# strukturag/libheif

Measured on NVIDIA H100. Metric: megapixels/sec HEIC-grid decode->RGB, higher is better.
Workload: dtype u8

## Files before the change

### libheif_b200/csrc/b200_hevc.h

```cpp
#pragma once
#include "b200_internal.h"
#include "b200_hevc_types.h"
#include "b200_hevc_syntax.h"
#include "b200_hevc_scaling.h"
#include <vector>

namespace b200 {

struct ParseLimits { uint64_t max_image_size_pixels = 0; };

struct PictureHeaders {
  PicDesc desc;
  syn::SeqParams sp;
  std::vector<SliceInfo> slices;
  std::vector<syn::Substream> subs;
  std::vector<uint8_t> rbsp;
  std::vector<uint16_t> ctu_slice;
  int colour_primaries = 2, transfer_characteristics = 2, matrix_coefficients = 2, full_range = 0;
  bool scaling_enabled = false;
  sl::Factors scaling;
};

struct ParsedPicture {
  PictureHeaders hdr;
// ... 15 lines not shown
  const int8_t* qp8; const uint8_t* edge8;
  const uint8_t* scaling;
  unsigned int* progress;
  const unsigned int* entropy_progress;
  int blocks_per_sm;
  unsigned int* ticket;
  unsigned int* error_flag;
  const uint2* row_list;
  int nrows;
  int wide_samples;
  int max_log2_ctb;
};
enum { MAX_CHUNKS = 16 };
struct EntropyPic { syn::SeqParams sp; syn::PicBuffers pb; uint32_t progress_base, sub_base; };
struct EntropyBatch {
  const EntropyPic* pics; int npics;
  const syn::Substream* subs;
  int nsubs;
  unsigned int* queue; unsigned int* qhead; unsigned int* qtail; unsigned int* deps;
  unsigned int* progress; unsigned int* sub_done; unsigned int* error_flag;
  int blocks_per_sm;
  int common;
};
int launch_entropy(const EntropyBatch& b, cudaStream_t s, int* resident_warps = nullptr);
int launch_entropy_gate(const EntropyBatch& b, int resident_warps, cudaStream_t s);
int launch_entropy_stats(const EntropyBatch& b, unsigned long long* out2, cudaStream_t s);
int launch_recon(const DeviceBatch& b, cudaStream_t s);
int launch_deblock(const DeviceBatch& b, const PicDesc* host_pics, cudaStream_t s);
int launch_sao(const DeviceBatch& b, const PicDesc* host_pics, cudaStream_t s, int* launches = nullptr);

}
```

### libheif_b200/csrc/b200_hevc_decode.cu

```cuda
#include "b200_hevc.h"
#include "b200_staging.h"
#include <chrono>
#include <functional>
#include <memory>
#include <mutex>
#include <string>
#include <unistd.h>

using namespace b200;

namespace {

double now_ms() { return std::chrono::duration<double, std::milli>(std::chrono::steady_clock::now().time_since_epoch()).count(); }

struct ScratchLayout {
  size_t n_rows = 0, n_subs = 0;
  static constexpr size_t error_flag = 1, progress = 2;
  size_t tickets() const { return progress + 3 * n_rows; }
  size_t sync_size() const { return tickets() + MAX_CHUNKS; }
  static constexpr size_t entropy_progress = 1;
  size_t sub_done() const { return entropy_progress + n_rows; }
  size_t esync_size() const { return sub_done() + n_subs; }
  static constexpr size_t qhead = 0, qtail = 1, queue = 2;
  size_t deps() const { return queue + n_subs; }
// ... 23 lines not shown
  bool device_front_end = false;
  size_t n_subs = 0;
  bool any_tiles = false;
  bool all_common = false;
  int bands = 0;
};

enum { OVERLAP_K0_BLOCKS_PER_SM = 3, OVERLAP_K1_BLOCKS_PER_SM = 2 };

struct LaunchPlan {
  int bands = 1, rows_per_band = 1;
  bool banded = false;
  bool overlap = false;
  bool tail = false;
  int k0_blocks_per_sm = 0, k1_blocks_per_sm = 0;
  bool common_k0 = false;
};

int sm_count() { int dev = 0, sms = 148; cudaGetDevice(&dev); cudaDeviceGetAttribute(&sms, cudaDevAttrMultiProcessorCount, dev); return sms; }

LaunchPlan plan_launches(const BatchShape& b, bool hook, const Overrides& env) {
  LaunchPlan p;
  const bool devfe = b.device_front_end;
  const bool one_wave = devfe && (env.overlap == Overrides::AUTO ? b.n_subs <= (size_t)sm_count() * 16
                                                                  : env.overlap == Overrides::ON);
  p.bands = b.bands;
  if (!p.bands) {
    p.bands = 1; p.rows_per_band = b.rows;
    if (b.rows >= 2 && (env.bands != Overrides::AUTO ? env.bands == Overrides::ON : hook && !one_wave)) {
      const int target = env.band_tiles > 0 ? env.band_tiles : (b.cols * b.rows + 1) / 2;
      int rpb = std::max(1, (target + b.cols / 2) / b.cols);
      if ((b.rows + rpb - 1) / rpb > MAX_CHUNKS) rpb = (b.rows + MAX_CHUNKS - 1) / MAX_CHUNKS;
      p.rows_per_band = rpb; p.bands = (b.rows + rpb - 1) / rpb;
    }
  }
  p.banded = p.bands > 1 && (hook || env.bands == Overrides::ON);
  p.overlap = !p.banded && one_wave;
  p.tail = devfe && env.overlap == Overrides::AUTO && env.tail && (!p.overlap || env.tail_force);
  if (p.tail) p.overlap = true;
  if (b.any_tiles) p.overlap = p.tail = false;
  if (p.overlap && !p.tail) { p.k0_blocks_per_sm = OVERLAP_K0_BLOCKS_PER_SM; p.k1_blocks_per_sm = OVERLAP_K1_BLOCKS_PER_SM; }
  p.common_k0 = b.all_common;
  return p;
}

}

// ... 706 lines not shown
```

### libheif_b200/csrc/b200_hevc_entropy.cu

```cuda
#include <cstdint>
#include <cstdlib>
namespace b200 { namespace syn {
__shared__ uint32_t s_kLps4[64];
__shared__ uint8_t s_kTransLps[64];
__shared__ uint8_t s_kNextState[256];
__shared__ unsigned long long s_kState[128];
__shared__ uint8_t s_kInitI[135];
__shared__ uint8_t s_kSigMap4[16];
__shared__ uint8_t s_kScanPos[3][16];
__shared__ uint8_t s_kScanInv[3][16];
__shared__ uint8_t s_kSbInv[4][3][64];
__shared__ uint8_t s_kSigCtx4[3][16];
__shared__ uint8_t s_kSigCtxN[3][4][16];
__shared__ uint8_t s_kChromaTab[4];
__shared__ uint8_t s_kScanX[4][3][64];
__shared__ uint8_t s_kScanY[4][3][64];
} }
#ifdef __CUDA_ARCH__
#define B200_T(name) s_##name
#endif
#include "b200_hevc.h"
static_assert(b200::syn::CTX_COUNT == 135, "s_kInitI above is sized for 135 context variables");

namespace b200 {
// ... 25 lines not shown
      if (e_ld_acquire(p) >= need) return;
      if ((++spins & 63u) != 0) continue;
      if (e_ld_acquire(error_flag)) return;
      if (spins > (1u << 23)) { atomicExch(error_flag, 3u); return; }
    }
  }
  __device__ void wait_row(int row, int need) { spin_until(progress + row, (unsigned)need, error_flag); }
  __device__ void publish_row(int row, int done) { e_st_release(progress + row, (unsigned)done); }
  __device__ void wait_substream(int idx) { spin_until(sub_done + idx, 1u, error_flag); }
  __device__ void finish_substream(int idx, int err) {
    e_st_release(sub_done + idx, 1u);
    if (err) atomicExch(error_flag, (unsigned)err);
  }
  __device__ void notify(int target) {
    if (target < 0) return;
    __threadfence();
    if (atomicSub(deps + target, 1u) == 1u) { const unsigned s = atomicAdd(qtail, 1u); e_st_release(queue + s, (unsigned)target + 1u); }
  }
};

#ifndef B200_ENTROPY_MIN_BLOCKS
#define B200_ENTROPY_MIN_BLOCKS 1
#endif
template <class Cfg>
__global__ void __launch_bounds__(EWARPS * 32, B200_ENTROPY_MIN_BLOCKS) hevc_entropy_kernel(const EntropyBatch b) {
  __shared__ __align__(8) syn::U2 s_ctx[EWARPS][syn::CTX_COUNT];
  __shared__ syn::DecoderT<Cfg> s_dec[EWARPS];
  for (int i = threadIdx.x; i < 64; i += blockDim.x) { syn::s_kLps4[i] = syn::d_kLps4[i]; syn::s_kTransLps[i] = syn::d_kTransLps[i]; }
  for (int i = threadIdx.x; i < syn::CTX_COUNT; i += blockDim.x) syn::s_kInitI[i] = syn::d_kInitI[i];
  for (int i = threadIdx.x; i < 256; i += blockDim.x) syn::s_kNextState[i] = syn::d_kNextState[i];
  for (int i = threadIdx.x; i < 128; i += blockDim.x) syn::s_kState[i] = syn::d_kState[i];
  for (int i = threadIdx.x; i < 16; i += blockDim.x) syn::s_kSigMap4[i] = syn::d_kSigMap4[i];
  for (int i = threadIdx.x; i < 48; i += blockDim.x) { (&syn::s_kScanPos[0][0])[i] = (&syn::d_kScanPos[0][0])[i]; (&syn::s_kScanInv[0][0])[i] = (&syn::d_kScanInv[0][0])[i]; (&syn::s_kSigCtx4[0][0])[i] = (&syn::d_kSigCtx4[0][0])[i]; }
  for (int i = threadIdx.x; i < 192; i += blockDim.x) (&syn::s_kSigCtxN[0][0][0])[i] = (&syn::d_kSigCtxN[0][0][0])[i];
  for (int i = threadIdx.x; i < 768; i += blockDim.x) (&syn::s_kSbInv[0][0][0])[i] = (&syn::d_kSbInv[0][0][0])[i];
  for (int i = threadIdx.x; i < 4; i += blockDim.x) syn::s_kChromaTab[i] = syn::d_kChromaTab[i];
  for (int i = threadIdx.x; i < 4 * 3 * 64; i += blockDim.x) { (&syn::s_kScanX[0][0][0])[i] = (&syn::d_kScanX[0][0][0])[i]; (&syn::s_kScanY[0][0][0])[i] = (&syn::d_kScanY[0][0][0])[i]; }
  __syncthreads();
  if ((threadIdx.x & 31) != 0) return;
  const int slot_w = threadIdx.x >> 5;
  const syn::CtxPtr ctx = (syn::CtxPtr)__cvta_generic_to_shared(s_ctx[slot_w]);
  for (;;) {
    const unsigned slot = atomicAdd(b.qhead, 1u);
    if (slot >= (unsigned)b.nsubs) break;
    unsigned item = e_ld_acquire(b.queue + slot);
    if (!item) {
      unsigned ns = 500, spins = 0;
      for (;;) {
        __nanosleep(ns); if (ns < 16000) ns <<= 1;
        if ((item = e_ld_acquire(b.queue + slot)) != 0u) break;
        if ((++spins & 31u) != 0) continue;
        if (e_ld_acquire(b.error_flag)) return;
        if (spins > (1u << 22)) { atomicExch(b.error_flag, 3u); return; }
      }
    }
    const syn::Substream& gs = b.subs[item - 1u];
    const EntropyPic& ep = b.pics[gs.pic];
    DevSync sync;
    sync.progress = b.progress + ep.progress_base; sync.sub_done = b.sub_done + ep.sub_base; sync.error_flag = b.error_flag;
    sync.queue = b.queue; sync.qtail = b.qtail; sync.deps = b.deps;
    sync.dense_tu = sync.dense_coef = sync.dense_tu_cap = sync.dense_coef_cap = 0; sync.end_bit_position = 0;
    syn::run_substream<Cfg>(s_dec[slot_w], ep.sp, ep.pb, b.subs + ep.sub_base, (int)(item - 1u - ep.sub_base), ctx, sync);
  }
}

__global__ void entropy_stats_kernel(const EntropyBatch b, unsigned long long* out2) {
  const int pi = blockIdx.y;
  const EntropyPic& ep = b.pics[pi];
  const int nctb = ep.sp.wctb * ep.sp.hctb;
  unsigned long long tus = 0, coefs = 0;
  for (int a = blockIdx.x * blockDim.x + threadIdx.x; a < nctb; a += gridDim.x * blockDim.x) {
    const CtuInfo ci = ep.pb.ctus[a];
    tus += ci.tu_count;
    for (unsigned k = 0; k < ci.tu_count; k++) { const TuCmd t = ep.pb.tus[ci.tu_start + k]; coefs += (t.w3 & 0x7ff) + ((t.w3 >> 11) & 0x3ff) + ((t.w3 >> 21) & 0x3ff); }
  }
  atomicAdd(out2, tus); atomicAdd(out2 + 1, coefs);
}

__global__ void entropy_gate_kernel(const unsigned* qhead, unsigned need, const unsigned* error_flag) {
  for (unsigned spins = 0; spins < 2000000u; spins++) {
    if (e_ld_acquire(qhead) >= need || e_ld_acquire(error_flag)) return;
    __nanosleep(1000);
  }
}

int launch_entropy_gate(const EntropyBatch& b, int resident_warps, cudaStream_t s) {
  if (b.nsubs <= 0 || resident_warps <= 0) return B200_OK;
  entropy_gate_kernel<<<1, 1, 0, s>>>(b.qhead, (unsigned)(resident_warps < b.nsubs ? resident_warps : b.nsubs), b.error_flag);
  cudaError_t e = cudaGetLastError();
  if (e != cudaSuccess) return set_error(B200_E_CUDA, "entropy gate launch: %s", cudaGetErrorString(e));
  return B200_OK;
}

int launch_entropy(const EntropyBatch& b, cudaStream_t s, int* resident_warps) {
  if (resident_warps) *resident_warps = 0;
  if (b.nsubs <= 0) return B200_OK;
  int dev = 0, sms = 148; cudaGetDevice(&dev); cudaDeviceGetAttribute(&sms, cudaDevAttrMultiProcessorCount, dev);
  auto kern = b.common ? hevc_entropy_kernel<syn::CfgCommon> : hevc_entropy_kernel<syn::CfgRuntime>;
  int occ = 1; cudaOccupancyMaxActiveBlocksPerMultiprocessor(&occ, kern, EWARPS * 32, 0);
  if (occ < 1) occ = 1;
  if (b.blocks_per_sm > 0 && b.blocks_per_sm < occ) occ = b.blocks_per_sm;
  const int want = (b.nsubs + EWARPS - 1) / EWARPS;
  const int grid = want < sms * occ ? want : sms * occ;
  if (resident_warps) *resident_warps = grid * EWARPS;
  kern<<<grid, EWARPS * 32, 0, s>>>(b);
  cudaError_t e = cudaGetLastError();
  if (e != cudaSuccess) return set_error(B200_E_CUDA, "entropy launch: %s", cudaGetErrorString(e));
  return B200_OK;
}

int launch_entropy_stats(const EntropyBatch& b, unsigned long long* out2, cudaStream_t s) {
  if (b.npics <= 0) return B200_OK;
  entropy_stats_kernel<<<dim3(8, b.npics), 128, 0, s>>>(b, out2);
  cudaError_t e = cudaGetLastError();
  if (e != cudaSuccess) return set_error(B200_E_CUDA, "entropy stats launch: %s", cudaGetErrorString(e));
  return B200_OK;
}

}
```

### libheif_b200/csrc/b200_hevc_syntax.h

```cpp
#pragma once
#include <cstdint>
#include <cstring>
#include "b200_hevc_types.h"

#if defined(__CUDA_ARCH__) && !defined(B200_SYNTAX_HOST_ONLY)
#define B200_SYN_DEVICE 1
#endif
#if defined(__CUDACC__) && !defined(B200_SYNTAX_HOST_ONLY)
#define B200_HDN __host__ __device__ __noinline__
#define B200_NOUNROLL _Pragma("unroll 1")
#define B200_HD __host__ __device__
#define B200_HDI __host__ __device__ __forceinline__
#define B200_TABLE(type, name, dims, ...) static const type h_##name dims = __VA_ARGS__; static __device__ const type d_##name dims = __VA_ARGS__;
#else
#define B200_HDN
#define B200_NOUNROLL
#define B200_HD
#define B200_HDI inline
#define B200_TABLE(type, name, dims, ...) static const type h_##name dims = __VA_ARGS__;
#endif
#if defined(B200_SYN_DEVICE) && !defined(B200_T)
#define B200_T(name) d_##name
#endif
#ifdef B200_SYN_DEVICE
// ... 215 lines not shown
  }
}

enum { SYN_OK = 0, SYN_E_BITSTREAM = 1, SYN_E_OVERFLOW = 2 };

struct SaoRaw { int8_t type[3], band[3], eo[3]; int8_t off[3][4]; };

struct CfgRuntime { enum : int { chroma = -1, bd = -1, log2_min_cb = -1, log2_min_tb = -1, log2_max_tb = -1, transform_skip = -1, cu_qp_delta = -1, sign_hiding = -1, sao_enabled = -1, wpp = -1, dense = -1, pcm = -1, tq_bypass = -1, tiles = -1 }; };
struct CfgCommon { enum : int { chroma = 1, bd = 8, log2_min_cb = 3, log2_min_tb = 2, log2_max_tb = 5, transform_skip = 0, cu_qp_delta = 1, sign_hiding = 1, sao_enabled = 1, wpp = 1, dense = 0, pcm = 0, tq_bypass = 0, tiles = 0 }; };
B200_HD inline bool matches_common(const SeqParams& q) {
  return q.chroma == 1 && q.bd == 8 && q.log2_min_cb == 3 && q.log2_min_tb == 2 && q.log2_max_tb == 5 && !q.transform_skip && q.cu_qp_delta == 1 && q.sign_hiding == 1 &&
         q.sao_enabled == 1 && q.wpp == 1 && q.dense == 0 && !q.pcm && !q.tq_bypass && !q.tiles;
}
#define B200_SPC(f) ((int)Cfg::f >= 0 ? (int)Cfg::f : (int)sp->f)
#define B200_SPR(f) ((int)Cfg::f >= 0 ? (int)Cfg::f : (int)sp.f)

template <class Cfg>
struct DecoderT {
  const SeqParams* sp; PicBuffers pb; const Substream* ss;
  Cabac cabac; CabacStream stream; CtxPtr ctx;
  int is_dqp_coded, dqp_val, qpy_prev_qg, last_cu_qpy, first_qg, cur_qpy, err;
  int cu_bypass;
  uint32_t tu_n, coef_n, tu_cap, coef_cap;
  int cur_ctb_x, cur_ctb_y;
  int ctb_x0, ctb_y0, left_ok, up_ok;
  int left_lf, up_lf;
  struct Cu { int x0, y0, log2cb, nxn, lmode[4], cmode; int cmodes[4]; };

  B200_HD inline bool avail(int x, int y) const { return x >= ctb_x0 ? (y >= ctb_y0 ? true : up_ok != 0) : left_ok != 0; }
  B200_HD inline int ld_cell(const uint8_t* p, int y) const { return y >= ctb_y0 ? (int)*p : (int)B200_LD_SHARED(p); }

  B200_HDN int dbin(int ci) { return cabac.bin(ctx_at(ctx, ci), stream); }
  B200_HDN int dbypass() { return cabac.bypass(stream); }
  B200_HDN unsigned dbits(int k) { return cabac.bypass_bits(k, stream); }

  B200_HDN void parse_sao(int rx, int ry, CtuInfo& ci) {
    const int addr = ry * sp->wctb + rx;
    B200_NOUNROLL for (int c = 0; c < 3; c++) { ci.sao[c].type = 0; ci.sao[c].band_or_class = 0; B200_NOUNROLL for (int k = 0; k < 4; k++) ci.sao[c].offset[k] = 0; }
    if (!ss->sao_luma && !ss->sao_chroma) return;
    int ml = 0, mu = 0;
    if (left_ok) ml = dbin(CTX_SAO_MERGE);
    if (up_ok && !ml) mu = dbin(CTX_SAO_MERGE);
    if (ml || mu) {
      const unsigned long long* o = reinterpret_cast<const unsigned long long*>(pb.ctus[ml ? addr - 1 : addr - sp->wctb].sao);
      unsigned long long* dsto = reinterpret_cast<unsigned long long*>(ci.sao);
      B200_NOUNROLL for (int c = 0; c < 3; c++) dsto[c] = B200_LD_SHARED(o + c);
// ... 13 lines not shown
        B200_NOUNROLL for (int i = 0; i < 4; i++) ci.sao[c].offset[i] = (int8_t)clip3(-128, 127, av[i] * (1 << sc));
      } else {
        if (c < 2) ci.sao[c].band_or_class = (uint8_t)dbits(2); else ci.sao[2].band_or_class = ci.sao[1].band_or_class;
        ci.sao[c].offset[0] = (int8_t)clip3(-128, 127, av[0] << sc); ci.sao[c].offset[1] = (int8_t)clip3(-128, 127, av[1] << sc);
        ci.sao[c].offset[2] = (int8_t)clip3(-128, 127, -(av[2] << sc)); ci.sao[c].offset[3] = (int8_t)clip3(-128, 127, -(av[3] << sc));
      }
    }
  }

  B200_HDN void derive_qpy(int xcb, int ycb) {
    const int mask = (1 << sp->qg_log2) - 1, xqg = xcb & ~mask, yqg = ycb & ~mask, cm = ~((1 << sp->log2ctb) - 1);
    int qa = qpy_prev_qg, qb = qpy_prev_qg;
    if (avail(xqg - 1, yqg) && ((xqg - 1) & cm) == (xqg & cm)) qa = pb.qp8[(yqg >> 3) * sp->w8 + ((xqg - 1) >> 3)];
    if (avail(xqg, yqg - 1) && ((yqg - 1) & cm) == (yqg & cm)) qb = pb.qp8[((yqg - 1) >> 3) * sp->w8 + (xqg >> 3)];
    const int pred = (qa + qb + 1) >> 1, qbd = 6 * (B200_SPC(bd) - 8);
    cur_qpy = ((pred + dqp_val + 52 + 2 * qbd) % (52 + qbd)) - qbd;
  }

  B200_HDN int residual(int log2n, int c, int mode, int& tskip) {
    const int n = 1 << log2n;
    Cabac cb_ = cabac; const CtxPtr cx = ctx;
    const int bypass_cu = B200_SPC(tq_bypass) && cu_bypass;
    const int sign_hiding = B200_SPC(sign_hiding) && !bypass_cu;
    CoefEntry* const coef_out = pb.coefs; uint32_t cn = coef_n; const uint32_t ccap = coef_cap;
    tskip = 0;
    if (B200_SPC(transform_skip) && log2n == 2 && !bypass_cu) tskip = cb_.bin(ctx_at(cx, CTX_TSKIP + (c ? 1 : 0)), stream);
    const int cmax = (log2n << 1) - 1;
    int off, shift;
    if (c == 0) { off = 3 * (log2n - 2) + ((log2n - 1) >> 2); shift = (log2n + 1) >> 2; } else { off = 15; shift = log2n - 2; }
    int lx = 0, ly = 0;
    B200_NOUNROLL for (int xy = 0; xy < 2; xy++) {
      const CtxPtr lc = ctx_at(cx, (xy ? CTX_LAST_Y : CTX_LAST_X) + off);
      int l = 0;
      CtxPtr a_cur = lc; U2 e_cur = ctx_ld(a_cur);
      B200_NOUNROLL while (l < cmax) {
        const CtxPtr a_next = ctx_at(lc, (l + 1) >> shift);
        U2 e_next = ctx_ld(a_next), ne;
        const int b = cb_.bin_e(e_cur, a_cur, stream, ne);
        if (!b) break;
        if (a_next == a_cur) e_next = ne;
        a_cur = a_next; e_cur = e_next; l++;
      }
      if (xy) ly = l; else lx = l;
    }
    B200_NOUNROLL for (int xy = 0; xy < 2; xy++) {
      int l = xy ? ly : lx;
      if (l > 3) { const int nb = (l >> 1) - 1; l = (1 << nb) * (2 + (l & 1)) + (int)cb_.bypass_bits(nb, stream); }
      if (xy) ly = l; else lx = l;
    }
    int scan = 0;
    if (log2n == 2 || (log2n == 3 && (c == 0 || B200_SPC(chroma) == 3))) { if (mode >= 6 && mode <= 14) scan = 2; else if (mode >= 22 && mode <= 30) scan = 1; }
    if (scan == 2) { const int t = lx; lx = ly; ly = t; }
    if (lx >= n || ly >= n) { err = SYN_E_BITSTREAM; cabac = cb_; return 0; }
    const int l2sb = log2n - 2;
    const uint8_t *sbx = B200_T(kScanX)[l2sb][scan], *sby = B200_T(kScanY)[l2sb][scan], *spos = B200_T(kScanPos)[scan];
    const int last_sb = B200_T(kSbInv)[l2sb][scan][((ly >> 2) << 3) + (lx >> 2)];
    const int last_pos = B200_T(kScanInv)[scan][((ly & 3) << 2) + (lx & 3)];
    uint64_t csbf = 0;
    int carry = 1, count = 0; bool first_done = false;
    const int nsbw = 1 << l2sb;
    const int dc_ctx = CTX_SIG + (c ? 27 : 0);
    const int sig_base = log2n == 2 ? dc_ctx : (c == 0 ? CTX_SIG + (log2n == 3 ? (scan == 0 ? 9 : 15) : 21) : CTX_SIG + 27 + (log2n == 3 ? 9 : 12));
    B200_NOUNROLL for (int i = last_sb; i >= 0; i--) {
      const int xs = sbx[i], ys = sby[i];
      const int right = (xs + 1 < nsbw) ? (int)((csbf >> (ys * 8 + xs + 1)) & 1) : 0;
      const int below = (ys + 1 < nsbw) ? (int)((csbf >> ((ys + 1) * 8 + xs)) & 1) : 0;
      int infer_dc = 0;
      if (i < last_sb && i > 0) { if (!cb_.bin(ctx_at(cx, CTX_CSBF + ((right | below) ? 1 : 0) + (c ? 2 : 0)), stream)) continue; infer_dc = 1; }
      csbf |= 1ull << (ys * 8 + xs);
      const TabPtr tab = log2n == 2 ? B200_TADDR(kSigCtx4) + 16 * scan : B200_TADDR(kSigCtxN) + (64 * scan + 16 * (right | (below << 1)));
      const CtxPtr cbase = ctx_at(cx, sig_base + ((c == 0 && log2n > 2 && (xs | ys)) ? 3 : 0));
      unsigned sig = 0;
      int k = 15;
      if (i == last_sb) { sig = 1u; k = last_pos - 1; }
      if (k >= 0) {
        const CtxPtr a0 = i == 0 ? ctx_at(cx, dc_ctx) : ctx_at(cbase, (int)tab_ld8(tab, 0));
        CtxPtr a_cur = k > 0 ? ctx_at(cbase, (int)tab_ld8(tab, k)) : a0;
        U2 e_cur = ctx_ld(a_cur);
        B200_NOUNROLL for (; k > 0; k--) {
          const CtxPtr a_next = k > 1 ? ctx_at(cbase, (int)tab_ld8(tab, k - 1)) : a0;
          U2 e_next = ctx_ld(a_next), ne;
          sig = (sig << 1) | (unsigned)cb_.bin_e(e_cur, a_cur, stream, ne);
          if (a_next == a_cur) e_next = ne;
          a_cur = a_next; e_cur = e_next;
        }
        if (infer_dc && !sig) sig = 1u;
        else { U2 ne; sig = (sig << 1) | (unsigned)cb_.bin_e(e_cur, a_cur, stream, ne); }
      }
      if (!sig) continue;
      unsigned g1 = 0;
      int g1ctx = 1, g2 = 0;
      int ctx_set = (i == 0 || c > 0) ? 0 : 2;
      if (first_done && carry == 0) ctx_set++;
      first_done = true;
      const int last_sig = hi_bit(sig), first_sig = lo_bit(sig);
      { unsigned m = sig; const CtxPtr gbase = ctx_at(cx, CTX_GT1 + ctx_set * 4 + (c ? 16 : 0));
        B200_NOUNROLL for (int ng1 = 0; m && ng1 < 8; ng1++) {
          const int kk = hi_bit(m); m ^= 1u << kk;
          if (cb_.bin(ctx_at(gbase, imin(3, g1ctx)), stream)) { g1 |= 1u << kk; g1ctx = 0; } else if (g1ctx > 0) g1ctx++;
        } }
      carry = g1ctx;
      const int last_g1 = g1 ? hi_bit(g1) : -1;
      const bool hidden = sign_hiding && (last_sig - first_sig > 3);
      if (last_g1 >= 0) g2 = cb_.bin(ctx_at(cx, CTX_GT2 + ctx_set + (c ? 4 : 0)), stream);
      const int nsign = pop_count(sig) - (hidden ? 1 : 0);
      const unsigned signs = cb_.bypass_bits(nsign, stream);
      int nsig = 0, sum = 0, rice = 0, sidx = nsign;
      B200_NOUNROLL for (unsigned m = sig; m; nsig++) {
        const int kk = hi_bit(m); m ^= 1u << kk;
        const int base = 1 + (int)((g1 >> kk) & 1) + (kk == last_g1 ? g2 : 0);
        int a = base;
        if (base == ((nsig < 8) ? ((kk == last_g1) ? 3 : 2) : 1)) {
          int pre = 0; B200_NOUNROLL while (pre < 32 && cb_.bypass(stream)) pre++;
          if (pre > 20) { err = SYN_E_BITSTREAM; cabac = cb_; coef_n = cn; return count; }
          const int rem = (pre <= 3 ? (pre << rice) : (((1 << (pre - 3)) + 3 - 1) << rice)) + (int)cb_.bypass_bits(pre <= 3 ? rice : pre - 3 + rice, stream);
          a = base + rem;
          if (a > 3 * (1 << rice)) rice = imin(rice + 1, 4);
        }
        int neg = 0;
        if (!hidden || kk != first_sig) { sidx--; neg = (int)((signs >> sidx) & 1); }
        int v = neg ? -a : a;
        if (hidden) { sum += a; if (kk == first_sig && (sum & 1)) v = -v; }
        if (cn >= ccap) { err = SYN_E_OVERFLOW; cabac = cb_; coef_n = cn; return count; }
        const int p = spos[kk];
        CoefEntry e; e.pos = (uint16_t)((((ys << 2) + (p >> 2)) << log2n) + (xs << 2) + (p & 3)); e.level = (int16_t)clip3(-32768, 32767, v);
        coef_out[cn++] = e; count++;
      }
    }
    cabac = cb_; coef_n = cn;
    return count;
  }

  B200_HDN void mark_tu(int x0, int y0, int log2n) {
    const SliceInfo& sl = pb.slices[ss->slice_idx];
    const int n8 = log2n > 3 ? 1 << (log2n - 3) : 1, bx = x0 >> 3, by = y0 >> 3;
    uint8_t left = 0, top = 0;
    if (!sl.deblocking_disabled) {
      if ((x0 & 7) == 0 && x0 > 0 && (x0 > ctb_x0 || left_lf)) left = 1;
      if ((y0 & 7) == 0 && y0 > 0 && (y0 > ctb_y0 || up_lf)) top = 2;
    }
    uint8_t* e = pb.edge8 + by * sp->w8 + bx;
    if (left) B200_NOUNROLL for (int y = 0; y < n8; y++) e[y * sp->w8] |= left;
    if (top) B200_NOUNROLL for (int x = 0; x < n8; x++) e[x] |= top;
  }

  B200_HDI void transform_unit(const Cu& cu, int x0, int y0, int log2n, int blk, int cbf_l, int cbf_cb, int cbf_cr, int pcb, int pcr) {
    const int cbf_c = B200_SPC(chroma) ? (log2n > 2 ? (cbf_cb | cbf_cr) : (pcb | pcr)) : 0;
    if ((cbf_l || cbf_c) && B200_SPC(cu_qp_delta) && !is_dqp_coded) {
      int v = 0;
      B200_NOUNROLL while (v < 5 && dbin(CTX_QP_DELTA + (v ? 1 : 0))) v++;
      if (v == 5) { int k = 0; B200_NOUNROLL while (k < 16 && dbypass()) { v += 1 << k; k++; } v += (int)dbits(k); }
      if (v && dbypass()) v = -v;
      { const int half = 3 * (B200_SPC(bd) - 8); if (v < -(26 + half) || v > 25 + half) { err = SYN_E_BITSTREAM; return; } }
      is_dqp_coded = 1; dqp_val = v;
      derive_qpy(cu.x0, cu.y0);
    }
    const int pu = cu.nxn ? ((y0 >= cu.y0 + (1 << (cu.log2cb - 1))) ? 2 : 0) + ((x0 >= cu.x0 + (1 << (cu.log2cb - 1))) ? 1 : 0) : 0;
    const int lmode = cu.lmode[pu];
    const uint32_t coef0 = coef_n;
    int ts_l = 0, ts_cb = 0, ts_cr = 0, nl = 0, ncb = 0, ncr = 0;
    int chroma_here = 0, ccb = 0, ccr = 0;
    if (B200_SPC(chroma)) {
      if (log2n > 2) { chroma_here = 1; ccb = cbf_cb; ccr = cbf_cr; }
      else if (blk == 3) { chroma_here = 1; ccb = pcb; ccr = pcr; }
    }
    B200_NOUNROLL for (int c = 0; c < 3; c++) {
      const int coded = c == 0 ? cbf_l : (c == 1 ? ccb : ccr);
      if (!coded) continue;
      int ts = 0;
      const int cnt = residual(c == 0 ? log2n : (log2n > 2 ? log2n - 1 : 2), c, c == 0 ? lmode : cu.cmode, ts);
      if (c == 0) { nl = cnt; ts_l = ts; } else if (c == 1) { ncb = cnt; ts_cb = ts; } else { ncr = cnt; ts_cr = ts; }
    }
    mark_tu(x0, y0, log2n);
    if (tu_n >= tu_cap) { err = SYN_E_OVERFLOW; return; }
    TuCmd t;
    t.w0 = (uint32_t)(x0 >> 2) | ((uint32_t)(y0 >> 2) << 12) | ((uint32_t)(log2n - 2) << 24) | ((uint32_t)cbf_l << 26) | ((uint32_t)ccb << 27) |
           ((uint32_t)ccr << 28) | ((uint32_t)chroma_here << 29) | ((uint32_t)ts_l << 30) | ((uint32_t)ts_cb << 31);
    t.w1 = (uint32_t)lmode | ((uint32_t)cu.cmode << 6) | ((uint32_t)(cur_qpy + 64) << 12) | ((uint32_t)ts_cr << 20) | ((B200_SPC(tq_bypass) && cu_bypass) ? 1u << 22 : 0u);
    t.w2 = coef0;
    t.w3 = (uint32_t)nl | ((uint32_t)ncb << 11) | ((uint32_t)ncr << 21);
    pb.tus[tu_n++] = t;
  }

  B200_HD static inline int zx(unsigned i) { i &= 0x55u; i = (i | (i >> 1)) & 0x33u; i = (i | (i >> 2)) & 0x0fu; return (int)i; }
  B200_HD static inline int node_depth(unsigned i, int levels) { const int up = i ? lo_bit(i) >> 1 : levels; return levels - imin(up, levels); }

  B200_HDI void transform_tree(const Cu& cu, int max_depth) {
    const int levels = cu.log2cb - 2, total = 1 << (2 * levels);
    unsigned cbm = 0, crm = 0;
    B200_NOUNROLL for (int j = 0; j < total && !err;) {
      int depth = node_depth((unsigned)j, levels);
      B200_NOUNROLL for (;;) {
        const int log2n = cu.log2cb - depth;
        const int x0 = cu.x0 + (zx((unsigned)j) << 2), y0 = cu.y0 + (zx((unsigned)j >> 1) << 2);
        const int blk = depth ? (j >> (2 * (levels - depth))) & 3 : 0;
        const int pcb = depth ? (int)((cbm >> (depth - 1)) & 1) : 0, pcr = depth ? (int)((crm >> (depth - 1)) & 1) : 0;
        int split;
        if (log2n <= B200_SPC(log2_max_tb) && log2n > B200_SPC(log2_min_tb) && depth < max_depth && !(cu.nxn && depth == 0)) split = dbin(CTX_SPLIT_TR + 5 - log2n);
        else split = (log2n > B200_SPC(log2_max_tb) || (cu.nxn && depth == 0)) ? 1 : 0;
        if (split && log2n <= 2) { err = SYN_E_BITSTREAM; break; }
        int cb = 0, cr = 0;
        if (B200_SPC(chroma)) {
          if (log2n > 2) {
// ... 189 lines not shown
    if (B200_SPC(pcm) && !cu.nxn && log2cb >= sp->log2_min_pcm && log2cb <= sp->log2_max_pcm && cabac.terminate(stream)) { pcm_unit(x0, y0, log2cb, depth); return; }
    const int np = cu.nxn ? 4 : 1, pbs = cu.nxn ? n / 2 : n;
    int prev[4], mi[4] = {0, 0, 0, 0}, rem[4] = {0, 0, 0, 0};
    B200_NOUNROLL for (int i = 0; i < np; i++) prev[i] = dbin(CTX_PREV_INTRA);
    B200_NOUNROLL for (int i = 0; i < np; i++) { if (prev[i]) { mi[i] = dbypass(); if (mi[i]) mi[i] += dbypass(); } else rem[i] = (int)dbits(5); }
    B200_NOUNROLL for (int i = 0; i < np; i++) {
      const int px = x0 + (i & 1) * pbs, py = y0 + (i >> 1) * pbs;
      const int m = luma_mode(px, py, prev[i], mi[i], rem[i]);
      cu.lmode[i] = m;
      B200_NOUNROLL for (int yy = 0; yy < pbs; yy += 4) B200_NOUNROLL for (int xx = 0; xx < pbs; xx += 4) pb.ipm4[((py + yy) >> 2) * sp->w4 + ((px + xx) >> 2)] = (uint8_t)m;
    }
    if (B200_SPC(chroma) >= 2) chroma_modes_x(cu, np);
    else if (B200_SPC(chroma)) {
      int v = 4; if (dbin(CTX_CHROMA_PRED)) v = (int)dbits(2);
      if (v == 4) cu.cmode = cu.lmode[0]; else { cu.cmode = B200_T(kChromaTab)[v]; if (cu.cmode == cu.lmode[0]) cu.cmode = 34; }
    }
    B200_NOUNROLL for (int yy = 0; yy < n; yy += 8) B200_NOUNROLL for (int xx = 0; xx < n; xx += 8) pb.cd8[((y0 + yy) >> 3) * sp->w8 + ((x0 + xx) >> 3)] = (uint8_t)depth;
    if (!B200_SPC(cu_qp_delta)) cur_qpy = ss->slice_qp; else derive_qpy(x0, y0);
    if (B200_SPC(chroma) >= 2) transform_tree_x(cu, sp->max_th_depth_intra + cu.nxn); else transform_tree(cu, sp->max_th_depth_intra + cu.nxn);
    B200_NOUNROLL for (int yy = 0; yy < n; yy += 8) B200_NOUNROLL for (int xx = 0; xx < n; xx += 8) pb.qp8[((y0 + yy) >> 3) * sp->w8 + ((x0 + xx) >> 3)] = (int8_t)cur_qpy;
    last_cu_qpy = cur_qpy;
  }

  B200_HDI void coding_quadtree(int xc, int yc) {
    const int log2min = B200_SPC(log2_min_cb), levels = sp->log2ctb - log2min, total = 1 << (2 * levels);
    B200_NOUNROLL for (int i = 0; i < total && !err;) {
      int depth = node_depth((unsigned)i, levels);
      B200_NOUNROLL for (;;) {
        const int log2cb = sp->log2ctb - depth, n = 1 << log2cb;
        const int x0 = xc + (zx((unsigned)i) << log2min), y0 = yc + (zx((unsigned)i >> 1) << log2min);
        if (x0 >= sp->W || y0 >= sp->H) { i += 1 << (2 * (levels - depth)); break; }
        int split;
        if (x0 + n <= sp->W && y0 + n <= sp->H && log2cb > log2min) {
          int inc = 0;
          if (avail(x0 - 1, y0) && (int)pb.cd8[(y0 >> 3) * sp->w8 + ((x0 - 1) >> 3)] > depth) inc++;
          if (avail(x0, y0 - 1) && ld_cell(pb.cd8 + ((y0 - 1) >> 3) * sp->w8 + (x0 >> 3), y0 - 1) > depth) inc++;
          split = dbin(CTX_SPLIT_CU + inc);
        } else split = log2cb > log2min;
        if (B200_SPC(cu_qp_delta) && log2cb >= sp->qg_log2) {
          is_dqp_coded = 0; dqp_val = 0;
          if (!split || log2cb == sp->qg_log2) { if (first_qg) { qpy_prev_qg = ss->slice_qp; first_qg = 0; } else qpy_prev_qg = last_cu_qpy; }
        }
        if (split) { depth++; continue; }
        coding_unit(x0, y0, log2cb, depth);
        i += 1 << (2 * (levels - depth));
        break;
      }
    }
  }

  B200_HDN void decode_ctb(int addr) {
    const int rx = addr % sp->wctb, ry = addr / sp->wctb;
    cur_ctb_x = rx; cur_ctb_y = ry;
    ctb_x0 = rx << sp->log2ctb; ctb_y0 = ry << sp->log2ctb;
    left_ok = rx > 0 && pb.ctu_slice[addr - 1] == (uint16_t)ss->slice_idx;
    up_ok = ry > 0 && pb.ctu_slice[addr - sp->wctb] == (uint16_t)ss->slice_idx;
    {
      const SliceInfo& cs = pb.slices[ss->slice_idx];
      left_lf = left_ok; up_lf = up_ok;
      if (rx > 0 && !left_ok) { const SliceInfo& o = pb.slices[pb.ctu_slice[addr - 1]]; left_lf = (o.slice_id == cs.slice_id || cs.lf_across_slices) && (o.tile_id == cs.tile_id || cs.lf_across_tiles); }
      if (ry > 0 && !up_ok) { const SliceInfo& o = pb.slices[pb.ctu_slice[addr - sp->wctb]]; up_lf = (o.slice_id == cs.slice_id || cs.lf_across_slices) && (o.tile_id == cs.tile_id || cs.lf_across_tiles); } }
    CtuInfo& ci = pb.ctus[addr];
    ci.slice_idx = (uint16_t)ss->slice_idx;
    if (!B200_SPC(dense)) { tu_n = (uint32_t)addr * (uint32_t)sp->tu_slots; tu_cap = tu_n + (uint32_t)sp->tu_slots; coef_n = (uint32_t)addr * (uint32_t)sp->coef_slots; coef_cap = coef_n + (uint32_t)sp->coef_slots; }
    const uint32_t t0 = tu_n;
    if (B200_SPC(sao_enabled)) parse_sao(rx, ry, ci);
    else for (int c = 0; c < 3; c++) { ci.sao[c].type = 0; ci.sao[c].band_or_class = 0; B200_NOUNROLL for (int k = 0; k < 4; k++) ci.sao[c].offset[k] = 0; }
    { const int b0x = rx << (sp->log2ctb - 3), b0y = ry << (sp->log2ctb - 3), nb = 1 << (sp->log2ctb - 3);
      B200_NOUNROLL for (int y = 0; y < nb && b0y + y < sp->h8; y++) B200_NOUNROLL for (int x = 0; x < nb && b0x + x < sp->w8; x++) pb.edge8[(b0y + y) * sp->w8 + b0x + x] = 0; }
    coding_quadtree(rx << sp->log2ctb, ry << sp->log2ctb);
    ci.tu_start = t0; ci.tu_count = (uint16_t)(tu_n - t0);
  }
};

typedef DecoderT<CfgRuntime> Decoder;

template <class Cfg, class Sync>
B200_HD int run_substream(DecoderT<Cfg>& d, const SeqParams& sp, const PicBuffers& pb, const Substream* all, int index, CtxPtr ctx, Sync& sync) {
  const Substream& ss = all[index];
  d.sp = &sp; d.pb = pb; d.ss = &ss; d.ctx = ctx; d.err = SYN_OK;
  d.is_dqp_coded = 0; d.dqp_val = 0; d.qpy_prev_qg = ss.slice_qp; d.last_cu_qpy = ss.slice_qp; d.first_qg = 1; d.cur_qpy = ss.slice_qp; d.cu_bypass = 0;
  d.tu_n = 0; d.coef_n = 0; d.tu_cap = 0; d.coef_cap = 0;
  if (B200_SPR(dense)) {
    d.tu_n = sync.dense_tu; d.coef_n = sync.dense_coef; d.tu_cap = sync.dense_tu_cap; d.coef_cap = sync.dense_coef_cap;
  }
  const int rx0 = (int)(ss.ctb_begin % (uint32_t)sp.wctb), ry0 = (int)(ss.ctb_begin / (uint32_t)sp.wctb);
  if (ss.prev >= 0) {
    sync.wait_substream(ss.prev);
    const uint8_t* st = pb.end_state + (size_t)ss.prev * CTX_STRIDE;
    B200_NOUNROLL for (int i = 0; i < CTX_COUNT; i++) ctx_st(ctx_at(ctx, i), tab_ld64(B200_TADDR(kState), (int)B200_LD_SHARED(st + i) & 127));
    d.last_cu_qpy = (int)(int8_t)B200_LD_SHARED(st + CTX_COUNT); d.first_qg = 0;
  }
  if (ss.init_contexts) init_contexts(ctx, ss.slice_qp);
  if (B200_SPR(wpp) && rx0 == 0 && (!ss.init_contexts || ss.prev >= 0) && ss.ctb_begin != ss.slice_addr_rs) {
    const int xn = 1 << sp.log2ctb, yn = (ry0 - 1) << sp.log2ctb;
    bool tr = ry0 > 0 && xn < sp.W && pb.ctu_slice[(ry0 - 1) * sp.wctb + 1] == (uint16_t)ss.slice_idx;
    (void)yn;
    if (tr) { sync.wait_row(ry0 - 1, 2); const uint8_t* st = pb.wpp_ctx + (size_t)(ry0 - 1) * CTX_STRIDE; B200_NOUNROLL for (int i = 0; i < CTX_COUNT; i++) ctx_st(ctx_at(ctx, i), tab_ld64(B200_TADDR(kState), (int)B200_LD_SHARED(st + i) & 127)); }
    else if (ss.prev < 0) init_contexts(ctx, ss.slice_qp);
    d.first_qg = 1;
  }
  d.stream.d = pb.rbsp; d.stream.size = pb.rbsp_size;
  d.cabac.start(d.stream, ss.byte_begin);
  const bool tiles = B200_SPR(tiles) != 0;
  int rx = rx0, ry = ry0;
  const uint32_t nctb = ss.ctb_end - ss.ctb_begin;
  B200_NOUNROLL for (uint32_t k = 0; k < nctb; k++, rx++) {
    if (rx == (int)ss.tile_x1) { rx = (int)ss.tile_x0; ry++; }
    const uint32_t a = (uint32_t)ry * (uint32_t)sp.wctb + (uint32_t)rx;
    if (ry > 0 && !tiles) sync.wait_row(ry - 1, rx + 1);
    if (B200_SPR(wpp) && rx == 0 && a != ss.ctb_begin) {
      d.first_qg = 1;
    }
    if (!B200_SPR(wpp) && rx == 0 && a != ss.ctb_begin) {  }
    d.decode_ctb((int)a);
    if (d.err) break;
    if (B200_SPR(wpp) && rx == 1) { uint8_t* st = pb.wpp_ctx + (size_t)ry * CTX_STRIDE; B200_NOUNROLL for (int i = 0; i < CTX_COUNT; i++) st[i] = (uint8_t)(ctx_ld(ctx_at(ctx, i)).y >> 24); }
    const int end = d.cabac.terminate(d.stream);
    const bool last = k + 1 == nctb;
    if (end != ((last && ss.last_of_segment) ? 1 : 0)) { d.err = SYN_E_BITSTREAM; break; }
    if (last && !ss.last_of_segment) { if (!d.cabac.terminate(d.stream)) { d.err = SYN_E_BITSTREAM; break; } }
    if (!tiles) sync.publish_row(ry, rx + 1);
    if (B200_SPR(wpp) && rx == 1) sync.notify(ss.wake_ctb2);
    if (d.cabac.pos > pb.rbsp_size + 64u) { d.err = SYN_E_BITSTREAM; break; }
  }
  { uint8_t* st = pb.end_state + (size_t)index * CTX_STRIDE; B200_NOUNROLL for (int i = 0; i < CTX_COUNT; i++) st[i] = (uint8_t)(ctx_ld(ctx_at(ctx, i)).y >> 24); st[CTX_COUNT] = (uint8_t)(int8_t)d.last_cu_qpy; }
  if (B200_SPR(dense)) { sync.dense_tu = d.tu_n; sync.dense_coef = d.coef_n; }
  sync.end_bit_position = d.cabac.bit_position();
  sync.finish_substream(index, d.err);
  if (!d.err) sync.notify(ss.wake_end);
  return d.err;
}

}
}
```

Measured before the change: 3691.

## Cut entropy kernel register pressure and raise occupancy for common config

The entropy kernel's register footprint is reduced in several ways. Per-warp sync state moves to shared memory, and live locals in residual coding are dropped: the coefficient counter is derived from indices, scan tables go through tab pointers, and quadtree levels are recomputed. TU fields are packed directly into the command word, and the loop re-reads state from the decoder object. The common-config kernel gets a min-blocks launch bound of 5, and the overlap one-wave threshold now uses the actual occupancy-derived warps per SM instead of a fixed 16. Forcing more blocks can cause spills, and the altered one-wave test can flip between overlap and banded launch plans.

```diff
diff --git a/libheif_b200/csrc/b200_hevc.h b/libheif_b200/csrc/b200_hevc.h
--- a/libheif_b200/csrc/b200_hevc.h
+++ b/libheif_b200/csrc/b200_hevc.h
@@ -61,6 +61,7 @@
   int blocks_per_sm;
   int common;
 };
+int entropy_warps_per_sm(bool common);
 int launch_entropy(const EntropyBatch& b, cudaStream_t s, int* resident_warps = nullptr);
 int launch_entropy_gate(const EntropyBatch& b, int resident_warps, cudaStream_t s);
 int launch_entropy_stats(const EntropyBatch& b, unsigned long long* out2, cudaStream_t s);
diff --git a/libheif_b200/csrc/b200_hevc_decode.cu b/libheif_b200/csrc/b200_hevc_decode.cu
--- a/libheif_b200/csrc/b200_hevc_decode.cu
+++ b/libheif_b200/csrc/b200_hevc_decode.cu
@@ -69,7 +69,7 @@
 LaunchPlan plan_launches(const BatchShape& b, bool hook, const Overrides& env) {
   LaunchPlan p;
   const bool devfe = b.device_front_end;
-  const bool one_wave = devfe && (env.overlap == Overrides::AUTO ? b.n_subs <= (size_t)sm_count() * 16
+  const bool one_wave = devfe && (env.overlap == Overrides::AUTO ? b.n_subs <= (size_t)sm_count() * entropy_warps_per_sm(b.all_common)
                                                                   : env.overlap == Overrides::ON);
   p.bands = b.bands;
   if (!p.bands) {
diff --git a/libheif_b200/csrc/b200_hevc_entropy.cu b/libheif_b200/csrc/b200_hevc_entropy.cu
--- a/libheif_b200/csrc/b200_hevc_entropy.cu
+++ b/libheif_b200/csrc/b200_hevc_entropy.cu
@@ -71,10 +71,16 @@
 #ifndef B200_ENTROPY_MIN_BLOCKS
 #define B200_ENTROPY_MIN_BLOCKS 1
 #endif
+#ifndef B200_ENTROPY_MAX_BLOCKS_PER_SM
+#define B200_ENTROPY_MAX_BLOCKS_PER_SM 0
+#endif
+template <class Cfg> constexpr int entropy_min_blocks() { return B200_ENTROPY_MIN_BLOCKS; }
+template <> constexpr int entropy_min_blocks<syn::CfgCommon>() { return B200_ENTROPY_MIN_BLOCKS > 5 ? B200_ENTROPY_MIN_BLOCKS : 5; }
 template <class Cfg>
-__global__ void __launch_bounds__(EWARPS * 32, B200_ENTROPY_MIN_BLOCKS) hevc_entropy_kernel(const EntropyBatch b) {
+__global__ void __launch_bounds__(EWARPS * 32, entropy_min_blocks<Cfg>()) hevc_entropy_kernel(const EntropyBatch b) {
   __shared__ __align__(8) syn::U2 s_ctx[EWARPS][syn::CTX_COUNT];
   __shared__ syn::DecoderT<Cfg> s_dec[EWARPS];
+  __shared__ DevSync s_sync[EWARPS];
   for (int i = threadIdx.x; i < 64; i += blockDim.x) { syn::s_kLps4[i] = syn::d_kLps4[i]; syn::s_kTransLps[i] = syn::d_kTransLps[i]; }
   for (int i = threadIdx.x; i < syn::CTX_COUNT; i += blockDim.x) syn::s_kInitI[i] = syn::d_kInitI[i];
   for (int i = threadIdx.x; i < 256; i += blockDim.x) syn::s_kNextState[i] = syn::d_kNextState[i];
@@ -105,7 +111,7 @@
     }
     const syn::Substream& gs = b.subs[item - 1u];
     const EntropyPic& ep = b.pics[gs.pic];
-    DevSync sync;
+    DevSync& sync = s_sync[slot_w];
     sync.progress = b.progress + ep.progress_base; sync.sub_done = b.sub_done + ep.sub_base; sync.error_flag = b.error_flag;
     sync.queue = b.queue; sync.qtail = b.qtail; sync.deps = b.deps;
     sync.dense_tu = sync.dense_coef = sync.dense_tu_cap = sync.dense_coef_cap = 0; sync.end_bit_position = 0;
@@ -141,13 +147,22 @@
   return B200_OK;
 }
 
+static int entropy_blocks_per_sm(bool common) {
+  auto kern = common ? hevc_entropy_kernel<syn::CfgCommon> : hevc_entropy_kernel<syn::CfgRuntime>;
+  int occ = 1; cudaOccupancyMaxActiveBlocksPerMultiprocessor(&occ, kern, EWARPS * 32, 0);
+  if (occ < 1) occ = 1;
+  if (B200_ENTROPY_MAX_BLOCKS_PER_SM > 0 && occ > B200_ENTROPY_MAX_BLOCKS_PER_SM) occ = B200_ENTROPY_MAX_BLOCKS_PER_SM;
+  return occ;
+}
+
+int entropy_warps_per_sm(bool common) { return entropy_blocks_per_sm(common) * EWARPS; }
+
 int launch_entropy(const EntropyBatch& b, cudaStream_t s, int* resident_warps) {
   if (resident_warps) *resident_warps = 0;
   if (b.nsubs <= 0) return B200_OK;
   int dev = 0, sms = 148; cudaGetDevice(&dev); cudaDeviceGetAttribute(&sms, cudaDevAttrMultiProcessorCount, dev);
   auto kern = b.common ? hevc_entropy_kernel<syn::CfgCommon> : hevc_entropy_kernel<syn::CfgRuntime>;
-  int occ = 1; cudaOccupancyMaxActiveBlocksPerMultiprocessor(&occ, kern, EWARPS * 32, 0);
-  if (occ < 1) occ = 1;
+  int occ = entropy_blocks_per_sm(b.common != 0);
   if (b.blocks_per_sm > 0 && b.blocks_per_sm < occ) occ = b.blocks_per_sm;
   const int want = (b.nsubs + EWARPS - 1) / EWARPS;
   const int grid = want < sms * occ ? want : sms * occ;
diff --git a/libheif_b200/csrc/b200_hevc_syntax.h b/libheif_b200/csrc/b200_hevc_syntax.h
--- a/libheif_b200/csrc/b200_hevc_syntax.h
+++ b/libheif_b200/csrc/b200_hevc_syntax.h
@@ -261,6 +261,7 @@
   int is_dqp_coded, dqp_val, qpy_prev_qg, last_cu_qpy, first_qg, cur_qpy, err;
   int cu_bypass;
   uint32_t tu_n, coef_n, tu_cap, coef_cap;
+  uint32_t ctb_tu0;
   int cur_ctb_x, cur_ctb_y;
   int ctb_x0, ctb_y0, left_ok, up_ok;
   int left_lf, up_lf;
@@ -320,7 +321,7 @@
     Cabac cb_ = cabac; const CtxPtr cx = ctx;
     const int bypass_cu = B200_SPC(tq_bypass) && cu_bypass;
     const int sign_hiding = B200_SPC(sign_hiding) && !bypass_cu;
-    CoefEntry* const coef_out = pb.coefs; uint32_t cn = coef_n; const uint32_t ccap = coef_cap;
+    uint32_t cn = coef_n;
     tskip = 0;
     if (B200_SPC(transform_skip) && log2n == 2 && !bypass_cu) tskip = cb_.bin(ctx_at(cx, CTX_TSKIP + (c ? 1 : 0)), stream);
     const int cmax = (log2n << 1) - 1;
@@ -351,28 +352,27 @@
     if (scan == 2) { const int t = lx; lx = ly; ly = t; }
     if (lx >= n || ly >= n) { err = SYN_E_BITSTREAM; cabac = cb_; return 0; }
     const int l2sb = log2n - 2;
-    const uint8_t *sbx = B200_T(kScanX)[l2sb][scan], *sby = B200_T(kScanY)[l2sb][scan], *spos = B200_T(kScanPos)[scan];
+    const TabPtr sbx = B200_TADDR(kScanX) + 64 * (3 * l2sb + scan), sby = B200_TADDR(kScanY) + 64 * (3 * l2sb + scan), spos = B200_TADDR(kScanPos) + 16 * scan;
     const int last_sb = B200_T(kSbInv)[l2sb][scan][((ly >> 2) << 3) + (lx >> 2)];
     const int last_pos = B200_T(kScanInv)[scan][((ly & 3) << 2) + (lx & 3)];
     uint64_t csbf = 0;
-    int carry = 1, count = 0; bool first_done = false;
-    const int nsbw = 1 << l2sb;
-    const int dc_ctx = CTX_SIG + (c ? 27 : 0);
-    const int sig_base = log2n == 2 ? dc_ctx : (c == 0 ? CTX_SIG + (log2n == 3 ? (scan == 0 ? 9 : 15) : 21) : CTX_SIG + 27 + (log2n == 3 ? 9 : 12));
+    int carry = 1;
+    const int sig_base = log2n == 2 ? CTX_SIG + (c ? 27 : 0) : (c == 0 ? CTX_SIG + (log2n == 3 ? (scan == 0 ? 9 : 15) : 21) : CTX_SIG + 27 + (log2n == 3 ? 9 : 12));
     B200_NOUNROLL for (int i = last_sb; i >= 0; i--) {
-      const int xs = sbx[i], ys = sby[i];
-      const int right = (xs + 1 < nsbw) ? (int)((csbf >> (ys * 8 + xs + 1)) & 1) : 0;
-      const int below = (ys + 1 < nsbw) ? (int)((csbf >> ((ys + 1) * 8 + xs)) & 1) : 0;
+      const int xs = (int)tab_ld8(sbx, i), ys = (int)tab_ld8(sby, i);
+      const int right = ((xs + 1) >> l2sb) == 0 ? (int)((csbf >> (ys * 8 + xs + 1)) & 1) : 0;
+      const int below = ((ys + 1) >> l2sb) == 0 ? (int)((csbf >> ((ys + 1) * 8 + xs)) & 1) : 0;
+      const bool is_last = csbf == 0;
       int infer_dc = 0;
-      if (i < last_sb && i > 0) { if (!cb_.bin(ctx_at(cx, CTX_CSBF + ((right | below) ? 1 : 0) + (c ? 2 : 0)), stream)) continue; infer_dc = 1; }
+      if (!is_last && i > 0) { if (!cb_.bin(ctx_at(cx, CTX_CSBF + ((right | below) ? 1 : 0) + (c ? 2 : 0)), stream)) continue; infer_dc = 1; }
       csbf |= 1ull << (ys * 8 + xs);
       const TabPtr tab = log2n == 2 ? B200_TADDR(kSigCtx4) + 16 * scan : B200_TADDR(kSigCtxN) + (64 * scan + 16 * (right | (below << 1)));
       const CtxPtr cbase = ctx_at(cx, sig_base + ((c == 0 && log2n > 2 && (xs | ys)) ? 3 : 0));
       unsigned sig = 0;
       int k = 15;
-      if (i == last_sb) { sig = 1u; k = last_pos - 1; }
+      if (is_last) { sig = 1u; k = last_pos - 1; }
       if (k >= 0) {
-        const CtxPtr a0 = i == 0 ? ctx_at(cx, dc_ctx) : ctx_at(cbase, (int)tab_ld8(tab, 0));
+        const CtxPtr a0 = i == 0 ? ctx_at(cx, CTX_SIG + (c ? 27 : 0)) : ctx_at(cbase, (int)tab_ld8(tab, 0));
         CtxPtr a_cur = k > 0 ? ctx_at(cbase, (int)tab_ld8(tab, k)) : a0;
         U2 e_cur = ctx_ld(a_cur);
         B200_NOUNROLL for (; k > 0; k--) {
@@ -389,8 +389,7 @@
       unsigned g1 = 0;
       int g1ctx = 1, g2 = 0;
       int ctx_set = (i == 0 || c > 0) ? 0 : 2;
-      if (first_done && carry == 0) ctx_set++;
-      first_done = true;
+      if (carry == 0) ctx_set++;
       const int last_sig = hi_bit(sig), first_sig = lo_bit(sig);
       { unsigned m = sig; const CtxPtr gbase = ctx_at(cx, CTX_GT1 + ctx_set * 4 + (c ? 16 : 0));
         B200_NOUNROLL for (int ng1 = 0; m && ng1 < 8; ng1++) {
@@ -410,7 +409,7 @@
         int a = base;
         if (base == ((nsig < 8) ? ((kk == last_g1) ? 3 : 2) : 1)) {
           int pre = 0; B200_NOUNROLL while (pre < 32 && cb_.bypass(stream)) pre++;
-          if (pre > 20) { err = SYN_E_BITSTREAM; cabac = cb_; coef_n = cn; return count; }
+          if (pre > 20) { err = SYN_E_BITSTREAM; cabac = cb_; const int count = (int)(cn - coef_n); coef_n = cn; return count; }
           const int rem = (pre <= 3 ? (pre << rice) : (((1 << (pre - 3)) + 3 - 1) << rice)) + (int)cb_.bypass_bits(pre <= 3 ? rice : pre - 3 + rice, stream);
           a = base + rem;
           if (a > 3 * (1 << rice)) rice = imin(rice + 1, 4);
@@ -419,13 +418,15 @@
         if (!hidden || kk != first_sig) { sidx--; neg = (int)((signs >> sidx) & 1); }
         int v = neg ? -a : a;
         if (hidden) { sum += a; if (kk == first_sig && (sum & 1)) v = -v; }
-        if (cn >= ccap) { err = SYN_E_OVERFLOW; cabac = cb_; coef_n = cn; return count; }
-        const int p = spos[kk];
+        if (cn >= coef_cap) { err = SYN_E_OVERFLOW; cabac = cb_; const int count = (int)(cn - coef_n); coef_n = cn; return count; }
+        const int p = (int)tab_ld8(spos, kk);
         CoefEntry e; e.pos = (uint16_t)((((ys << 2) + (p >> 2)) << log2n) + (xs << 2) + (p & 3)); e.level = (int16_t)clip3(-32768, 32767, v);
-        coef_out[cn++] = e; count++;
-      }
-    }
-    cabac = cb_; coef_n = cn;
+        pb.coefs[cn++] = e;
+      }
+    }
+    cabac = cb_;
+    const int count = (int)(cn - coef_n);
+    coef_n = cn;
     return count;
   }
 
@@ -456,27 +457,28 @@
     const int pu = cu.nxn ? ((y0 >= cu.y0 + (1 << (cu.log2cb - 1))) ? 2 : 0) + ((x0 >= cu.x0 + (1 << (cu.log2cb - 1))) ? 1 : 0) : 0;
     const int lmode = cu.lmode[pu];
     const uint32_t coef0 = coef_n;
-    int ts_l = 0, ts_cb = 0, ts_cr = 0, nl = 0, ncb = 0, ncr = 0;
     int chroma_here = 0, ccb = 0, ccr = 0;
     if (B200_SPC(chroma)) {
       if (log2n > 2) { chroma_here = 1; ccb = cbf_cb; ccr = cbf_cr; }
       else if (blk == 3) { chroma_here = 1; ccb = pcb; ccr = pcr; }
     }
-    B200_NOUNROLL for (int c = 0; c < 3; c++) {
-      const int coded = c == 0 ? cbf_l : (c == 1 ? ccb : ccr);
-      if (!coded) continue;
-      int ts = 0;
-      const int cnt = residual(c == 0 ? log2n : (log2n > 2 ? log2n - 1 : 2), c, c == 0 ? lmode : cu.cmode, ts);
-      if (c == 0) { nl = cnt; ts_l = ts; } else if (c == 1) { ncb = cnt; ts_cb = ts; } else { ncr = cnt; ts_cr = ts; }
-    }
-    mark_tu(x0, y0, log2n);
-    if (tu_n >= tu_cap) { err = SYN_E_OVERFLOW; return; }
     TuCmd t;
     t.w0 = (uint32_t)(x0 >> 2) | ((uint32_t)(y0 >> 2) << 12) | ((uint32_t)(log2n - 2) << 24) | ((uint32_t)cbf_l << 26) | ((uint32_t)ccb << 27) |
-           ((uint32_t)ccr << 28) | ((uint32_t)chroma_here << 29) | ((uint32_t)ts_l << 30) | ((uint32_t)ts_cb << 31);
-    t.w1 = (uint32_t)lmode | ((uint32_t)cu.cmode << 6) | ((uint32_t)(cur_qpy + 64) << 12) | ((uint32_t)ts_cr << 20) | ((B200_SPC(tq_bypass) && cu_bypass) ? 1u << 22 : 0u);
+           ((uint32_t)ccr << 28) | ((uint32_t)chroma_here << 29);
+    t.w1 = (uint32_t)lmode | ((uint32_t)cu.cmode << 6) | ((B200_SPC(tq_bypass) && cu_bypass) ? 1u << 22 : 0u);
     t.w2 = coef0;
-    t.w3 = (uint32_t)nl | ((uint32_t)ncb << 11) | ((uint32_t)ncr << 21);
+    t.w3 = 0;
+    B200_NOUNROLL for (int c = 0; c < 3; c++) {
+      if (!((t.w0 >> (26 + c)) & 1u)) continue;
+      const int l2 = (int)((t.w0 >> 24) & 3u) + 2;
+      int ts = 0;
+      const int cnt = residual(c == 0 ? l2 : (l2 > 2 ? l2 - 1 : 2), c, (int)((t.w1 >> (c == 0 ? 0 : 6)) & 63u), ts);
+      t.w3 |= (uint32_t)cnt << (c == 0 ? 0 : (c == 1 ? 11 : 21));
+      if (c == 0) t.w0 |= (uint32_t)ts << 30; else if (c == 1) t.w0 |= (uint32_t)ts << 31; else t.w1 |= (uint32_t)ts << 20;
+    }
+    mark_tu((int)(t.w0 & 0xfffu) << 2, (int)((t.w0 >> 12) & 0xfffu) << 2, (int)((t.w0 >> 24) & 3u) + 2);
+    if (tu_n >= tu_cap) { err = SYN_E_OVERFLOW; return; }
+    t.w1 |= (uint32_t)(cur_qpy + 64) << 12;
     pb.tus[tu_n++] = t;
   }
 
@@ -712,14 +714,15 @@
     last_cu_qpy = cur_qpy;
   }
 
-  B200_HDI void coding_quadtree(int xc, int yc) {
-    const int log2min = B200_SPC(log2_min_cb), levels = sp->log2ctb - log2min, total = 1 << (2 * levels);
-    B200_NOUNROLL for (int i = 0; i < total && !err;) {
-      int depth = node_depth((unsigned)i, levels);
+  B200_HD inline int cq_levels() const { return sp->log2ctb - B200_SPC(log2_min_cb); }
+  B200_HDI void coding_quadtree() {
+    const int log2min = B200_SPC(log2_min_cb);
+    B200_NOUNROLL for (int i = 0; i < (1 << (2 * cq_levels())) && !err;) {
+      int depth = node_depth((unsigned)i, cq_levels());
       B200_NOUNROLL for (;;) {
         const int log2cb = sp->log2ctb - depth, n = 1 << log2cb;
-        const int x0 = xc + (zx((unsigned)i) << log2min), y0 = yc + (zx((unsigned)i >> 1) << log2min);
-        if (x0 >= sp->W || y0 >= sp->H) { i += 1 << (2 * (levels - depth)); break; }
+        const int x0 = ctb_x0 + (zx((unsigned)i) << log2min), y0 = ctb_y0 + (zx((unsigned)i >> 1) << log2min);
+        if (x0 >= sp->W || y0 >= sp->H) { i += 1 << (2 * (cq_levels() - depth)); break; }
         int split;
         if (x0 + n <= sp->W && y0 + n <= sp->H && log2cb > log2min) {
           int inc = 0;
@@ -733,7 +736,7 @@
         }
         if (split) { depth++; continue; }
         coding_unit(x0, y0, log2cb, depth);
-        i += 1 << (2 * (levels - depth));
+        i += 1 << (2 * (cq_levels() - depth));
         break;
       }
     }
@@ -753,13 +756,14 @@
     CtuInfo& ci = pb.ctus[addr];
     ci.slice_idx = (uint16_t)ss->slice_idx;
     if (!B200_SPC(dense)) { tu_n = (uint32_t)addr * (uint32_t)sp->tu_slots; tu_cap = tu_n + (uint32_t)sp->tu_slots; coef_n = (uint32_t)addr * (uint32_t)sp->coef_slots; coef_cap = coef_n + (uint32_t)sp->coef_slots; }
-    const uint32_t t0 = tu_n;
+    ctb_tu0 = tu_n;
     if (B200_SPC(sao_enabled)) parse_sao(rx, ry, ci);
     else for (int c = 0; c < 3; c++) { ci.sao[c].type = 0; ci.sao[c].band_or_class = 0; B200_NOUNROLL for (int k = 0; k < 4; k++) ci.sao[c].offset[k] = 0; }
     { const int b0x = rx << (sp->log2ctb - 3), b0y = ry << (sp->log2ctb - 3), nb = 1 << (sp->log2ctb - 3);
       B200_NOUNROLL for (int y = 0; y < nb && b0y + y < sp->h8; y++) B200_NOUNROLL for (int x = 0; x < nb && b0x + x < sp->w8; x++) pb.edge8[(b0y + y) * sp->w8 + b0x + x] = 0; }
-    coding_quadtree(rx << sp->log2ctb, ry << sp->log2ctb);
-    ci.tu_start = t0; ci.tu_count = (uint16_t)(tu_n - t0);
+    coding_quadtree();
+    CtuInfo& ce = pb.ctus[cur_ctb_y * sp->wctb + cur_ctb_x];
+    ce.tu_start = ctb_tu0; ce.tu_count = (uint16_t)(tu_n - ctb_tu0);
   }
 };
 
@@ -794,31 +798,30 @@
   d.cabac.start(d.stream, ss.byte_begin);
   const bool tiles = B200_SPR(tiles) != 0;
   int rx = rx0, ry = ry0;
-  const uint32_t nctb = ss.ctb_end - ss.ctb_begin;
-  B200_NOUNROLL for (uint32_t k = 0; k < nctb; k++, rx++) {
-    if (rx == (int)ss.tile_x1) { rx = (int)ss.tile_x0; ry++; }
-    const uint32_t a = (uint32_t)ry * (uint32_t)sp.wctb + (uint32_t)rx;
+  B200_NOUNROLL for (uint32_t left = ss.ctb_end - ss.ctb_begin; left > 0; left--, rx++) {
+    if (rx == (int)d.ss->tile_x1) { rx = (int)d.ss->tile_x0; ry++; }
+    const uint32_t a = (uint32_t)ry * (uint32_t)d.sp->wctb + (uint32_t)rx;
     if (ry > 0 && !tiles) sync.wait_row(ry - 1, rx + 1);
-    if (B200_SPR(wpp) && rx == 0 && a != ss.ctb_begin) {
+    if (B200_SPR(wpp) && rx == 0 && a != d.ss->ctb_begin) {
       d.first_qg = 1;
     }
-    if (!B200_SPR(wpp) && rx == 0 && a != ss.ctb_begin) {  }
     d.decode_ctb((int)a);
     if (d.err) break;
-    if (B200_SPR(wpp) && rx == 1) { uint8_t* st = pb.wpp_ctx + (size_t)ry * CTX_STRIDE; B200_NOUNROLL for (int i = 0; i < CTX_COUNT; i++) st[i] = (uint8_t)(ctx_ld(ctx_at(ctx, i)).y >> 24); }
+    rx = d.cur_ctb_x; ry = d.cur_ctb_y;
+    if (B200_SPR(wpp) && rx == 1) { uint8_t* st = d.pb.wpp_ctx + (size_t)ry * CTX_STRIDE; B200_NOUNROLL for (int i = 0; i < CTX_COUNT; i++) st[i] = (uint8_t)(ctx_ld(ctx_at(d.ctx, i)).y >> 24); }
     const int end = d.cabac.terminate(d.stream);
-    const bool last = k + 1 == nctb;
-    if (end != ((last && ss.last_of_segment) ? 1 : 0)) { d.err = SYN_E_BITSTREAM; break; }
-    if (last && !ss.last_of_segment) { if (!d.cabac.terminate(d.stream)) { d.err = SYN_E_BITSTREAM; break; } }
+    const bool last = left == 1;
+    if (end != ((last && d.ss->last_of_segment) ? 1 : 0)) { d.err = SYN_E_BITSTREAM; break; }
+    if (last && !d.ss->last_of_segment) { if (!d.cabac.terminate(d.stream)) { d.err = SYN_E_BITSTREAM; break; } }
     if (!tiles) sync.publish_row(ry, rx + 1);
-    if (B200_SPR(wpp) && rx == 1) sync.notify(ss.wake_ctb2);
-    if (d.cabac.pos > pb.rbsp_size + 64u) { d.err = SYN_E_BITSTREAM; break; }
-  }
-  { uint8_t* st = pb.end_state + (size_t)index * CTX_STRIDE; B200_NOUNROLL for (int i = 0; i < CTX_COUNT; i++) st[i] = (uint8_t)(ctx_ld(ctx_at(ctx, i)).y >> 24); st[CTX_COUNT] = (uint8_t)(int8_t)d.last_cu_qpy; }
+    if (B200_SPR(wpp) && rx == 1) sync.notify(d.ss->wake_ctb2);
+    if (d.cabac.pos > d.pb.rbsp_size + 64u) { d.err = SYN_E_BITSTREAM; break; }
+  }
+  { uint8_t* st = d.pb.end_state + (size_t)index * CTX_STRIDE; B200_NOUNROLL for (int i = 0; i < CTX_COUNT; i++) st[i] = (uint8_t)(ctx_ld(ctx_at(d.ctx, i)).y >> 24); st[CTX_COUNT] = (uint8_t)(int8_t)d.last_cu_qpy; }
   if (B200_SPR(dense)) { sync.dense_tu = d.tu_n; sync.dense_coef = d.coef_n; }
   sync.end_bit_position = d.cabac.bit_position();
   sync.finish_substream(index, d.err);
-  if (!d.err) sync.notify(ss.wake_end);
+  if (!d.err) sync.notify(d.ss->wake_end);
   return d.err;
 }
 
```

Result: faster. 3941, median of 6 (+6.8%).
